# nmwsharp/diffusion-net

Hardware: AMD Instinct MI355X
Metric: vertices/sec fwd+bwd, C_width=128 K=128 (higher is better)
Workload: dtype f32; 1 GPU; train step (fwd+NLL+bwd+Adam) on a ragged batch of 16 meshes x ~10000 vertices per GPU, DiffusionNet C_in=3 C_out=8 C_width=128 K=128 N_block=4 outputs_at=faces dropout=on; meshes_per_gpu=16, verts_per_gpu_step=158481, parallelism=dp1, streams_per_gpu=1, step_mode=HIP-graph replay

## Files before the change

diffusion-net_amd/csrc/dn_tn_da.hip:

```cpp
#include "dn_common.h"
#include <string.h>

#define DN_DA_THREADS 512
#define DN_DA_KS 16
#define DN_DA_ROWB 576
#define DN_DA_PLANE (DN_DA_KS * DN_DA_ROWB)
#define DN_DA_BUF (6 * DN_DA_PLANE)
#define DN_DA_LDS (128 * 1024)

struct DaRegs {
    float4 dd, gx, gy;
    float live;
};

__device__ __forceinline__ void da_load(const DaArgs& g, long long r_beg, long long r_end, int step, int kr, int q, DaRegs& R) {
    const long long row = r_beg + (long long)step * DN_DA_KS + kr;
    const bool ok = row < r_end;
    const long long off = (ok ? row : r_beg) * 128 + 4 * q;
    R.live = ok ? 1.f : 0.f;
    R.dd = *reinterpret_cast<const float4*>(g.dd + off);
    R.gx = *reinterpret_cast<const float4*>(g.gx + off);
    R.gy = *reinterpret_cast<const float4*>(g.gy + off);
}

template <int NP>
__device__ __forceinline__ void da_put(unsigned char* planes, int off, float4 v, float s) {
    uint2 pl[NP];
    dn_split_f4<NP>(v, s, pl);
#pragma unroll
    for (int p = 0; p < NP; ++p) *reinterpret_cast<uint2*>(planes + p * DN_DA_PLANE + off) = pl[p];
}

template <int NP>
__device__ __forceinline__ void da_store(unsigned char* buf, int kr, int q, const DaRegs& R, float sa, float sb) {
    const float4 bx = dn_f4_scale(R.gx, R.live), by = dn_f4_scale(R.gy, R.live);
    const float4 ax = dn_f4_mul(R.dd, bx), ay = dn_f4_mul(R.dd, by);
    const int off = kr * DN_DA_ROWB + q * 8;
    da_put<NP>(buf, off, ax, sa);
    da_put<NP>(buf, off + 256, ay, sa);
    da_put<NP>(buf + 3 * DN_DA_PLANE, off, bx, sb);
    da_put<NP>(buf + 3 * DN_DA_PLANE, off + 256, by, sb);
}

__device__ __forceinline__ uint4 da_frag(const unsigned char* p) {
    const uint2 lo = dn_lds_tr16(p), hi = dn_lds_tr16(p + 4 * DN_DA_ROWB);
    return make_uint4(lo.x, lo.y, hi.x, hi.y);
}

template <int NP>
__device__ __forceinline__ void da_compute(const unsigned char* buf, int wr, int wc, int lane, f32x16 (&acc)[4][2]) {
    const int g = lane >> 4, c = lane & 15;
    const int lane_off = (8 * (g >> 1) + (c >> 2)) * DN_DA_ROWB + (16 * (g & 1) + 4 * (c & 3)) * 2;
    const unsigned char* sA = buf + lane_off + wr * 256;
    const unsigned char* sB = buf + 3 * DN_DA_PLANE + lane_off + wc * 128;
    uint4 b[NP][2];
#pragma unroll
    for (int p = 0; p < NP; ++p)
#pragma unroll
        for (int nt = 0; nt < 2; ++nt) b[p][nt] = da_frag(sB + p * DN_DA_PLANE + nt * 64);
#pragma unroll
    for (int mt = 0; mt < 4; ++mt) {
        uint4 a[NP];
#pragma unroll
        for (int p = 0; p < NP; ++p) a[p] = da_frag(sA + p * DN_DA_PLANE + mt * 64);
        constexpr int NPROD = NP == 3 ? 6 : 3;
        constexpr int PA[6] = {NP == 3 ? 1 : 0, NP == 3 ? 0 : 1, NP == 3 ? 2 : 0, 0, 1, 0};
        constexpr int PB[6] = {1, NP == 3 ? 2 : 0, 0, 1, 0, 0};
#pragma unroll
        for (int p = 0; p < NPROD; ++p)
#pragma unroll
            for (int nt = 0; nt < 2; ++nt) {
                if constexpr (NP == 3) acc[mt][nt] = dn_mfma_bf16(a[PA[p]], b[PB[p]][nt], acc[mt][nt]);
                else acc[mt][nt] = dn_mfma_f16(a[PA[p]], b[PB[p]][nt], acc[mt][nt]);
            }
    }
}

DN_CLK_DECLARE(tn_da)
template <int NP>
__global__ __launch_bounds__(DN_DA_THREADS) DN_WAVES_PER_EU(2) void tngemm_da_kernel(DaArgs g) {
    DN_CLK_STAMP(tn_da, 0);
    float sa = 1.f, sb = 1.f, so = 1.f;
    if constexpr (NP == 2) {
        sa = dn_pow2_scale(dn_amax_eval(g.a_amax));
        sb = dn_pow2_scale(dn_amax_eval(g.b_amax));
        so = (1.f / sa) * (1.f / sb);
    }
    DN_DYN_SMEM(smem_raw);
    unsigned char* smem = reinterpret_cast<unsigned char*>(smem_raw);
    const int tid = threadIdx.x, lane = tid & 63, wave = tid >> 6;
    const int wr = wave >> 2, wc = wave & 3;
    const int kr = tid >> 5, q = tid & 31;

    const long long r_beg = (long long)blockIdx.x * g.rows_per_wg;
    const long long r_end = (r_beg + g.rows_per_wg < g.V) ? r_beg + g.rows_per_wg : g.V;
    const int nsteps = r_end > r_beg ? (int)((r_end - r_beg + DN_DA_KS - 1) / DN_DA_KS) : 0;

    f32x16 acc[4][2];
#pragma unroll
    for (int i = 0; i < 4; ++i)
#pragma unroll
        for (int j = 0; j < 2; ++j)
#pragma unroll
            for (int r = 0; r < 16; ++r) acc[i][j][r] = 0.f;

    if (nsteps > 0) {
        DaRegs R0, R1;
        da_load(g, r_beg, r_end, 0, kr, q, R0);
        da_load(g, r_beg, r_end, 1, kr, q, R1);
        da_store<NP>(smem, kr, q, R0, sa, sb);
        da_load(g, r_beg, r_end, 2, kr, q, R0);
        __syncthreads();
        for (int s = 0; s < nsteps; s += 2) {
            da_store<NP>(smem + DN_DA_BUF, kr, q, R1, sa, sb);
            da_load(g, r_beg, r_end, s + 3, kr, q, R1);
            da_compute<NP>(smem, wr, wc, lane, acc);
            __syncthreads();
            if (s + 1 < nsteps) {
                da_store<NP>(smem, kr, q, R0, sa, sb);
                da_load(g, r_beg, r_end, s + 4, kr, q, R0);
                da_compute<NP>(smem + DN_DA_BUF, wr, wc, lane, acc);
                __syncthreads();
            }
        }
    }
    __syncthreads();

    float* ex = reinterpret_cast<float*>(smem);
    if (wc >= 2) {
        float* mine = ex + (size_t)(wr * 2 + (wc - 2)) * 8 * 16 * 64;
#pragma unroll
        for (int mt = 0; mt < 4; ++mt)
#pragma unroll
            for (int nt = 0; nt < 2; ++nt)
#pragma unroll
                for (int r = 0; r < 16; ++r) mine[((mt * 2 + nt) * 16 + r) * 64 + lane] = acc[mt][nt][r];
    }
    __syncthreads();
    if (wc < 2) {
        const float* theirs = ex + (size_t)((1 - wr) * 2 + wc) * 8 * 16 * 64;
        const float sgn = wr == 0 ? 1.f : -1.f;
        float* out = g.partial + ((long long)blockIdx.x * 2 + wr) * 128 * 128;
        const int li = lane & 31;
#pragma unroll
        for (int mt = 0; mt < 4; ++mt)
#pragma unroll
            for (int nt = 0; nt < 2; ++nt)
#pragma unroll
                for (int r = 0; r < 16; ++r) {
                    const int o = mt * 32 + dn_acc_row(r, lane), c = wc * 64 + nt * 32 + li;
                    const float v = acc[mt][nt][r] + sgn * theirs[((mt * 2 + nt) * 16 + r) * 64 + lane];
                    out[o * 128 + c] = NP == 2 ? v * so : v;
                }
    }
    DN_CLK_STAMP(tn_da, 1);
}

int dn_launch_tn_da(const float* dd, const float* gx, const float* gy, long long V, float* partial, int nwg, hipStream_t stream,
                    const float* dd_amax, const float* g_amax) {
    if (V <= 0 || nwg <= 0) return DN_ERR_BAD_MODE;
    DaArgs g;
    memset(&g, 0, sizeof(g));
    g.dd = dd; g.gx = gx; g.gy = gy; g.partial = partial; g.V = V;
    g.f16 = (dd_amax && g_amax) ? 1 : 0;
    g.a_amax.p[0] = dd_amax; g.a_amax.mul = g_amax; g.b_amax.p[0] = g_amax;
    const long long per = (V + nwg - 1) / nwg;
    g.rows_per_wg = (int)((per + DN_DA_KS - 1) / DN_DA_KS * DN_DA_KS);
#ifndef DN_EMULATE
    static unsigned long long lds_opt_in = 0;
    { const int oe_ = dn_lds_opt_in(reinterpret_cast<const void*>(&tngemm_da_kernel<3>), DN_DA_LDS, &lds_opt_in); if (oe_) return oe_; }
    static unsigned long long lds_opt_in2 = 0;
    { const int oe_ = dn_lds_opt_in(reinterpret_cast<const void*>(&tngemm_da_kernel<2>), DN_DA_LDS, &lds_opt_in2); if (oe_) return oe_; }
#endif
    dn_prof_begin(DN_K_TN_DA, stream);
    if (g.f16) DN_LAUNCH(tngemm_da_kernel<2>, dim3(nwg, 1, 1), dim3(DN_DA_THREADS, 1, 1), DN_DA_LDS, stream, g);
    else DN_LAUNCH(tngemm_da_kernel<3>, dim3(nwg, 1, 1), dim3(DN_DA_THREADS, 1, 1), DN_DA_LDS, stream, g);
    dn_prof_end(DN_K_TN_DA, stream, 8.0 * (double)V * 128.0 * 128.0, 4.0 * (3.0 * (double)V * 128.0 + 2.0 * nwg * 128.0 * 128.0));
    return (int)hipGetLastError();
}
```

diffusion-net_amd/csrc/dn_tn_tiles.h:

```cpp
#pragma once
#include "dn_common.h"

enum { DN_TN_PLAIN = 0, DN_TN_ROWSCALE = 1, DN_TN_COLSUM = 2, DN_TN_QA = 3 };

#define DN_TX_THREADS 512
#define DN_TX_ROWB 320
#define DN_TX_PLANE (DN_KB * DN_TX_ROWB)

struct TxRegs {
    float4 a[2], b[2], qa[2];
    float ma[2], mb[2];
};

template <int FLAVOR>
__device__ __forceinline__ void tx_load(const TnArgs& g, const DnTile& ch, int step, int kr0, bool a_ok, bool b_ok,
                                        const float* ap, const float* aq, int ald, const float* bp, int bld, TxRegs& R) {
#pragma unroll
    for (int i = 0; i < 2; ++i) {
        const int kr = step * DN_KB + kr0 + 16 * i;
        const bool kok = kr < ch.nrows;
        const long long row = (long long)ch.row0 + (kok ? kr : 0);
        R.ma[i] = (kok && a_ok) ? 1.f : 0.f;
        R.mb[i] = (kok && b_ok) ? 1.f : 0.f;
        R.a[i] = *reinterpret_cast<const float4*>(ap + row * ald);
        R.b[i] = *reinterpret_cast<const float4*>(bp + row * bld);
        if (FLAVOR == DN_TN_QA) R.qa[i] = *reinterpret_cast<const float4*>(aq + row * ald);
        if (FLAVOR == DN_TN_ROWSCALE) R.qa[i].x = g.b_rowscale[row];
    }
}

template <int NP = 3>
__device__ __forceinline__ void tx_put(unsigned char* planes, int off, float4 v, float s = 1.f) {
    uint2 pl[NP];
    dn_split_f4<NP>(v, s, pl);
#pragma unroll
    for (int p = 0; p < NP; ++p) *reinterpret_cast<uint2*>(planes + p * DN_TX_PLANE + off) = pl[p];
}

template <int FLAVOR, int NP = 3>
__device__ __forceinline__ void tx_store(unsigned char* sA, unsigned char* sB, int kr0, int q, const TxRegs& R, float4& csum,
                                         float sa = 1.f, float sb = 1.f) {
#pragma unroll
    for (int i = 0; i < 2; ++i) {
        float4 va = dn_f4_scale(R.a[i], R.ma[i]);
        const float4 vb = dn_f4_scale(R.b[i], FLAVOR == DN_TN_ROWSCALE ? R.mb[i] * R.qa[i].x : R.mb[i]);
        if (FLAVOR == DN_TN_QA) va = dn_f4_mul(va, R.qa[i]);
        if (FLAVOR == DN_TN_COLSUM) { csum.x += va.x; csum.y += va.y; csum.z += va.z; csum.w += va.w; }
        const int off = (kr0 + 16 * i) * DN_TX_ROWB + q * 8;
        tx_put<NP>(sA, off, va, sa);
        tx_put<NP>(sB, off, vb, sb);
    }
}

__device__ __forceinline__ uint4 tx_frag(const unsigned char* p) {
    const uint2 lo = dn_lds_tr16(p), hi = dn_lds_tr16(p + 4 * DN_TX_ROWB);
    return make_uint4(lo.x, lo.y, hi.x, hi.y);
}

template <int NP = 3>
__device__ __forceinline__ void tx_compute(const unsigned char* sA, const unsigned char* sB, int wr, int wc, int lane,
                                           f32x16 (&acc)[2]) {
    const int g = lane >> 4, c = lane & 15;
    const int lane_off = (8 * (g >> 1) + (c >> 2)) * DN_TX_ROWB + (16 * (g & 1) + 4 * (c & 3)) * 2;
#pragma unroll
    for (int s = 0; s < 2; ++s) {
        uint4 a[NP][2], b[NP];
#pragma unroll
        for (int p = 0; p < NP; ++p) {
            const int base = p * DN_TX_PLANE + s * 16 * DN_TX_ROWB + lane_off;
#pragma unroll
            for (int mt = 0; mt < 2; ++mt) a[p][mt] = tx_frag(sA + base + (wr * 64 + mt * 32) * 2);
            b[p] = tx_frag(sB + base + (wc * 32) * 2);
        }
        constexpr int NPROD = NP == 3 ? 6 : 3;
        constexpr int PA[6] = {NP == 3 ? 1 : 0, NP == 3 ? 0 : 1, NP == 3 ? 2 : 0, 0, 1, 0};
        constexpr int PB[6] = {1, NP == 3 ? 2 : 0, 0, 1, 0, 0};
#pragma unroll
        for (int p = 0; p < NPROD; ++p)
#pragma unroll
            for (int mt = 0; mt < 2; ++mt) {
                if constexpr (NP == 3) acc[mt] = dn_mfma_bf16(a[PA[p]][mt], b[PB[p]], acc[mt]);
                else acc[mt] = dn_mfma_f16(a[PA[p]][mt], b[PB[p]], acc[mt]);
            }
    }
}
```

diffusion-net_amd/csrc/dn_tngemm.hip:

```cpp
#include "dn_tn_tiles.h"
#include <string.h>

#define DN_TO 128

__device__ __forceinline__ float tn_elem(const TnSeg* s, int ns, long long row, int col) {
    int c = col;
    for (int i = 0; i < ns; ++i) {
        if (c < s[i].w) {
            const long long off = row * s[i].ld + c;
            float v = s[i].p[off];
            if (s[i].q) v *= s[i].q[off];
            return v;
        }
        c -= s[i].w;
    }
    return 0.f;
}


struct TnRegs {
    float4 a[4], b[4], qa[4];
    float ma[4], mb[4];
};

template <bool ALIGNED, int FLAVOR>
__device__ __forceinline__ void tn_load(const TnArgs& g, const DnTile& ch, int step, int kr0, int acol, int bcol, bool a_ok,
                                        bool b_ok, const float* ap, const float* aq, int ald, const float* bp, int bld,
                                        TnRegs& R) {
    if (ALIGNED) {
#pragma unroll
        for (int i = 0; i < 4; ++i) {
            const int kr = step * DN_KB + kr0 + 8 * i;
            const bool kok = kr < ch.nrows;
            const long long row = (long long)ch.row0 + (kok ? kr : 0);
            R.ma[i] = (kok && a_ok) ? 1.f : 0.f;
            R.mb[i] = (kok && b_ok) ? 1.f : 0.f;
            R.a[i] = *reinterpret_cast<const float4*>(ap + row * ald);
            R.b[i] = *reinterpret_cast<const float4*>(bp + row * bld);
            if (FLAVOR == DN_TN_QA) R.qa[i] = *reinterpret_cast<const float4*>(aq + row * ald);
            if (FLAVOR == DN_TN_ROWSCALE) R.qa[i].x = g.b_rowscale[row];
        }
    } else {
#pragma unroll
        for (int i = 0; i < 4; ++i) {
            const int kr = step * DN_KB + kr0 + 8 * i;
            const long long row = (long long)ch.row0 + kr;
            float e[4] = {0.f, 0.f, 0.f, 0.f}, f[4] = {0.f, 0.f, 0.f, 0.f};
            if (kr < ch.nrows) {
                const float rs = g.b_rowscale ? g.b_rowscale[row] : 1.f;
#pragma unroll
                for (int c = 0; c < 4; ++c) {
                    if (acol + c < g.M) e[c] = tn_elem(g.a, g.na, row, acol + c);
                    if (bcol + c < g.N) f[c] = tn_elem(g.b, g.nb, row, bcol + c) * rs;
                }
            }
            R.a[i] = make_float4(e[0], e[1], e[2], e[3]);
            R.b[i] = make_float4(f[0], f[1], f[2], f[3]);
            R.ma[i] = 1.f;
            R.mb[i] = 1.f;
            if (FLAVOR == DN_TN_QA) R.qa[i] = make_float4(1.f, 1.f, 1.f, 1.f);
            if (FLAVOR == DN_TN_ROWSCALE) R.qa[i].x = 1.f;
        }
    }
}

template <int FLAVOR>
__device__ __forceinline__ void tn_store(float* sA, float* sB, int kr0, int q, const TnRegs& R, float4& csum) {
#pragma unroll
    for (int i = 0; i < 4; ++i) {
        float4 va = dn_f4_scale(R.a[i], R.ma[i]);
        float4 vb = dn_f4_scale(R.b[i], FLAVOR == DN_TN_ROWSCALE ? R.mb[i] * R.qa[i].x : R.mb[i]);
        if (FLAVOR == DN_TN_QA) va = dn_f4_mul(va, R.qa[i]);
        if (FLAVOR == DN_TN_COLSUM) { csum.x += va.x; csum.y += va.y; csum.z += va.z; csum.w += va.w; }
        const int kr = kr0 + 8 * i;
        *reinterpret_cast<float4*>(&sA[kr * DN_TO + 4 * q]) = va;
        *reinterpret_cast<float4*>(&sB[kr * DN_TO + 4 * q]) = vb;
    }
}

__device__ __forceinline__ void tn_compute(const float* sA, const float* sB, int wr, int wc, int li, int ls, f32x16 (&acc)[2][2]) {
#pragma unroll
    for (int kg = 0; kg < 4; ++kg) {
        float af[2][4], bf[2][4];
#pragma unroll
        for (int t = 0; t < 4; ++t) {
            const int kr = 8 * kg + 4 * ls + t;
#pragma unroll
            for (int i = 0; i < 2; ++i) {
                af[i][t] = sA[kr * DN_TO + (wr * 2 + i) * 32 + li];
                bf[i][t] = sB[kr * DN_TO + (wc * 2 + i) * 32 + li];
            }
        }
#pragma unroll
        for (int t = 0; t < 4; ++t)
#pragma unroll
            for (int i = 0; i < 2; ++i)
#pragma unroll
                for (int j = 0; j < 2; ++j) acc[i][j] = dn_mfma(af[i][t], bf[j][t], acc[i][j]);
    }
}

template <bool ALIGNED, int FLAVOR>
__global__ __launch_bounds__(256) void tngemm_kernel(TnArgs g) {
    constexpr int SBUF = 2 * DN_KB * DN_TO;
    DN_DYN_SMEM(smem_raw);
    float* smem = reinterpret_cast<float*>(smem_raw);

    const int tid = threadIdx.x, lane = tid & 63, wave = tid >> 6;
    const int wr = wave >> 1, wc = wave & 1;
    const int li = lane & 31, ls = lane >> 5;
    const int n0 = blockIdx.y * DN_TO, m0 = blockIdx.z * DN_TO;
    const bool do_colsum = FLAVOR == DN_TN_COLSUM && blockIdx.y == 0;
    const bool wave_active = (m0 + wr * 64 < g.M) && (n0 + wc * 64 < g.N);

    f32x16 acc[2][2];
#pragma unroll
    for (int i = 0; i < 2; ++i)
#pragma unroll
        for (int j = 0; j < 2; ++j)
#pragma unroll
            for (int r = 0; r < 16; ++r) acc[i][j][r] = 0.f;

    const int q = tid & 31, kr0 = tid >> 5;
    const int acol = m0 + 4 * q, bcol = n0 + 4 * q;
    const float* ap = g.a[0].p; const float* aq = g.a[0].q ? g.a[0].q : g.a[0].p; int ald = g.a[0].ld;
    const float* bp = g.b[0].p; int bld = g.b[0].ld;
    const bool a_ok = acol < g.M, b_ok = bcol < g.N;
    if (ALIGNED) {
        int c = acol;
        for (int i = 0; i < g.na; ++i) {
            if (a_ok && c >= 0 && c < g.a[i].w) { ap = g.a[i].p + c; aq = (g.a[i].q ? g.a[i].q : g.a[i].p) + c; ald = g.a[i].ld; }
            c -= g.a[i].w;
        }
        c = bcol;
        for (int i = 0; i < g.nb; ++i) {
            if (b_ok && c >= 0 && c < g.b[i].w) { bp = g.b[i].p + c; bld = g.b[i].ld; }
            c -= g.b[i].w;
        }
    }
    float4 csum = dn_f4_zero();
    TnRegs R;

    const int c_beg = blockIdx.x * g.group;
    const int c_end = (c_beg + g.group < g.nchunks) ? c_beg + g.group : g.nchunks;
    for (int ci = c_beg; ci < c_end; ++ci) {
        const DnTile ch = g.chunks[ci];
        const int nsteps = (ch.nrows + DN_KB - 1) / DN_KB;
        tn_load<ALIGNED, FLAVOR>(g, ch, 0, kr0, acol, bcol, a_ok, b_ok, ap, aq, ald, bp, bld, R);
        tn_store<FLAVOR>(smem, smem + DN_KB * DN_TO, kr0, q, R, csum);
        if (nsteps > 1) tn_load<ALIGNED, FLAVOR>(g, ch, 1, kr0, acol, bcol, a_ok, b_ok, ap, aq, ald, bp, bld, R);
        __syncthreads();
        int st = 0;
        for (; st + 2 < nsteps; ++st) {
            float* cur = smem + (st & 1) * SBUF;
            float* nxt = smem + ((st & 1) ^ 1) * SBUF;
            tn_store<FLAVOR>(nxt, nxt + DN_KB * DN_TO, kr0, q, R, csum);
            tn_load<ALIGNED, FLAVOR>(g, ch, st + 2, kr0, acol, bcol, a_ok, b_ok, ap, aq, ald, bp, bld, R);
            tn_compute(cur, cur + DN_KB * DN_TO, wr, wc, li, ls, acc);
            __syncthreads();
        }
        if (st + 1 < nsteps) {
            float* cur = smem + (st & 1) * SBUF;
            float* nxt = smem + ((st & 1) ^ 1) * SBUF;
            tn_store<FLAVOR>(nxt, nxt + DN_KB * DN_TO, kr0, q, R, csum);
            tn_compute(cur, cur + DN_KB * DN_TO, wr, wc, li, ls, acc);
            __syncthreads();
            ++st;
        }
        {
            float* cur = smem + (st & 1) * SBUF;
            tn_compute(cur, cur + DN_KB * DN_TO, wr, wc, li, ls, acc);
            __syncthreads();
        }
    }
    float* out = g.partial + (long long)blockIdx.x * g.M * g.N;
#pragma unroll
    for (int i = 0; i < 2; ++i)
#pragma unroll
        for (int j = 0; j < 2; ++j) {
            if (!wave_active) continue;
            const int n = n0 + (wc * 2 + j) * 32 + li;
#pragma unroll
            for (int r = 0; r < 16; ++r) {
                const int m = m0 + (wr * 2 + i) * 32 + dn_acc_row(r, lane);
                if (m < g.M && n < g.N) out[(long long)m * g.N + n] = acc[i][j][r];
            }
        }
    if (do_colsum) {
        *reinterpret_cast<float4*>(&smem[kr0 * DN_TO + 4 * q]) = csum;
        __syncthreads();
        if (tid < DN_TO && m0 + tid < g.M) {
            float sum = 0.f;
#pragma unroll
            for (int k = 0; k < 8; ++k) sum += smem[k * DN_TO + tid];
            g.colsum[(long long)blockIdx.x * g.M + m0 + tid] = sum;
        }
    }
}

template <bool ALIGNED, int FLAVOR>
static int tn_launch(const TnArgs& g, dim3 grid, hipStream_t stream) {
    const size_t smem = (size_t)2 * 2 * DN_KB * DN_TO * sizeof(float);
    DN_LAUNCH((tngemm_kernel<ALIGNED, FLAVOR>), grid, dim3(256, 1, 1), smem, stream, g);
    return (int)hipGetLastError();
}

template <int FLAVOR, int NP>
__device__ __forceinline__ void tn_x3_body(const TnArgs& g, const int bx, const int by, const int bz) {
    float sa = 1.f, sb = 1.f, so = 1.f;
    if constexpr (NP == 2) {
        sa = dn_pow2_scale(dn_amax_eval(g.a_amax));
        sb = dn_pow2_scale(dn_amax_eval(g.b_amax));
        so = (1.f / sa) * (1.f / sb);
    }

    constexpr int SBUF = 6 * DN_TX_PLANE;
    DN_DYN_SMEM(smem_raw);
    unsigned char* smem = reinterpret_cast<unsigned char*>(smem_raw);

    const int tid = threadIdx.x, lane = tid & 63, wave = tid >> 6;
    const int wr = wave >> 2, wc = wave & 3;
    const int li = lane & 31;
    const int n0 = by * DN_TO, m0 = bz * DN_TO;
    const bool do_colsum = FLAVOR == DN_TN_COLSUM && by == 0;
    const bool wave_active = (m0 + wr * 64 < g.M) && (n0 + wc * 32 < g.N);

    f32x16 acc[2];
#pragma unroll
    for (int i = 0; i < 2; ++i)
#pragma unroll
        for (int r = 0; r < 16; ++r) acc[i][r] = 0.f;

    const int q = tid & 31, kr0 = tid >> 5;
    const int acol = m0 + 4 * q, bcol = n0 + 4 * q;
    const float* ap = g.a[0].p; const float* aq = g.a[0].q ? g.a[0].q : g.a[0].p; int ald = g.a[0].ld;
    const float* bp = g.b[0].p; int bld = g.b[0].ld;
    const bool a_ok = acol < g.M, b_ok = bcol < g.N;
    {
        int c = acol;
        for (int i = 0; i < g.na; ++i) {
            if (a_ok && c >= 0 && c < g.a[i].w) { ap = g.a[i].p + c; aq = (g.a[i].q ? g.a[i].q : g.a[i].p) + c; ald = g.a[i].ld; }
            c -= g.a[i].w;
        }
        c = bcol;
        for (int i = 0; i < g.nb; ++i) {
            if (b_ok && c >= 0 && c < g.b[i].w) { bp = g.b[i].p + c; bld = g.b[i].ld; }
            c -= g.b[i].w;
        }
    }
    float4 csum = dn_f4_zero();
    TxRegs R;

    const int c_beg = bx * g.group;
    const int c_end = (c_beg + g.group < g.nchunks) ? c_beg + g.group : g.nchunks;
    for (int ci = c_beg; ci < c_end; ++ci) {
        const DnTile ch = g.chunks[ci];
        const int nsteps = (ch.nrows + DN_KB - 1) / DN_KB;
        tx_load<FLAVOR>(g, ch, 0, kr0, a_ok, b_ok, ap, aq, ald, bp, bld, R);
        tx_store<FLAVOR, NP>(smem, smem + 3 * DN_TX_PLANE, kr0, q, R, csum, sa, sb);
        __syncthreads();
        for (int st = 0; st < nsteps; ++st) {
            if (st + 1 < nsteps) tx_load<FLAVOR>(g, ch, st + 1, kr0, a_ok, b_ok, ap, aq, ald, bp, bld, R);
            tx_compute<NP>(smem, smem + 3 * DN_TX_PLANE, wr, wc, lane, acc);
            __syncthreads();
            if (st + 1 < nsteps) {
                tx_store<FLAVOR, NP>(smem, smem + 3 * DN_TX_PLANE, kr0, q, R, csum, sa, sb);
                __syncthreads();
            }
        }
    }
    float* out = g.partial + (long long)bx * g.M * g.N;
    if (wave_active) {
        const int n = n0 + wc * 32 + li;
#pragma unroll
        for (int i = 0; i < 2; ++i)
#pragma unroll
            for (int r = 0; r < 16; ++r) {
                const int m = m0 + (wr * 2 + i) * 32 + dn_acc_row(r, lane);
                if (m < g.M && n < g.N) out[(long long)m * g.N + n] = NP == 2 ? acc[i][r] * so : acc[i][r];
            }
    }
    if (do_colsum) {
        float* red = reinterpret_cast<float*>(smem);
        *reinterpret_cast<float4*>(&red[kr0 * DN_TO + 4 * q]) = csum;
        __syncthreads();
        if (tid < DN_TO && m0 + tid < g.M) {
            float sum = 0.f;
#pragma unroll
            for (int k = 0; k < 16; ++k) sum += red[k * DN_TO + tid];
            g.colsum[(long long)bx * g.M + m0 + tid] = sum;
        }
    }
}

template <int FLAVOR, int NP>
__global__ __launch_bounds__(DN_TX_THREADS, 4) void tngemm_x3_kernel(TnArgs g) {
    int bx = blockIdx.x, by = blockIdx.y, bz = blockIdx.z;
    if (g.lin_ny > 0) {
        const int nt = g.lin_ny * g.lin_nz, nb = g.lin_nb, local = (int)blockIdx.x, nfull = nb & ~7;
        int tile;
        if (local < nfull * nt) { const int seq = local >> 3; bx = 8 * (seq / nt) + (local & 7); tile = seq % nt; }
        else { const int t = local - nfull * nt, rem = nb - nfull; bx = nfull + t % rem; tile = t / rem; }
        by = tile % g.lin_ny; bz = tile / g.lin_ny;
    }
    tn_x3_body<FLAVOR, NP>(g, bx, by, bz);
}
#define DN_TN_MULTI 3
struct TnMulti { TnArgs p[DN_TN_MULTI]; int first[DN_TN_MULTI + 1]; int nblk[DN_TN_MULTI]; int ny[DN_TN_MULTI]; int count; };
DN_CLK_DECLARE(tn_multi)
template <int FLAVOR, int NP>
__global__ __launch_bounds__(DN_TX_THREADS, 4) void tngemm_x3_multi_kernel(TnMulti mm) {
    DN_CLK_STAMP(tn_multi, 0);
    int pi = 0;
#pragma unroll
    for (int i = 1; i < DN_TN_MULTI; ++i) pi = (i < mm.count && (int)blockIdx.x >= mm.first[i]) ? i : pi;
    const int local = (int)blockIdx.x - mm.first[pi];
    if (pi == 0) tn_x3_body<FLAVOR, NP>(mm.p[0], local % mm.nblk[0], (local / mm.nblk[0]) % mm.ny[0], local / (mm.nblk[0] * mm.ny[0]));
    else if (pi == 1) tn_x3_body<FLAVOR, NP>(mm.p[1], local % mm.nblk[1], (local / mm.nblk[1]) % mm.ny[1], local / (mm.nblk[1] * mm.ny[1]));
    else tn_x3_body<FLAVOR, NP>(mm.p[2], local % mm.nblk[2], (local / mm.nblk[2]) % mm.ny[2], local / (mm.nblk[2] * mm.ny[2]));
    DN_CLK_STAMP(tn_multi, 1);
}

template <int FLAVOR, int NP>
static int tx_launch_np(const TnArgs& g, dim3 grid, hipStream_t stream) {
    const size_t smem = (size_t)6 * DN_TX_PLANE;
#ifndef DN_EMULATE
    static unsigned long long lds_opt_in = 0;
    { const int oe_ = dn_lds_opt_in(reinterpret_cast<const void*>(&tngemm_x3_kernel<FLAVOR, NP>), smem, &lds_opt_in); if (oe_) return oe_; }
#endif
    DN_LAUNCH((tngemm_x3_kernel<FLAVOR, NP>), grid, dim3(DN_TX_THREADS, 1, 1), smem, stream, g);
    return (int)hipGetLastError();
}
template <int FLAVOR>
static int tx_launch(const TnArgs& g, dim3 grid, hipStream_t stream) {
    return g.f16 ? tx_launch_np<FLAVOR, 2>(g, grid, stream) : tx_launch_np<FLAVOR, 3>(g, grid, stream);
}


int dn_launch_tngemm(const TnArgs& g_in, int nchunks, hipStream_t stream) {
    if (nchunks <= 0 || g_in.M <= 0 || g_in.N <= 0) return 0;
    TnArgs g = g_in;
    g.nchunks = nchunks;
    if (g.group < 1) g.group = 1;
    const int nblk = (nchunks + g.group - 1) / g.group;
    dim3 grid(nblk, (g.N + DN_TO - 1) / DN_TO, (g.M + DN_TO - 1) / DN_TO);
    bool has_qa = false;
    for (int i = 0; i < g.na; ++i) has_qa = has_qa || g.a[i].q != nullptr;
    for (int i = 0; i < g.nb; ++i) if (g.b[i].q) return DN_ERR_BAD_MODE;
    const int flavor = has_qa ? DN_TN_QA : (g.colsum ? DN_TN_COLSUM : (g.b_rowscale ? DN_TN_ROWSCALE : DN_TN_PLAIN));
    if ((has_qa && (g.colsum || g.b_rowscale)) || (g.colsum && g.b_rowscale)) return DN_ERR_BAD_MODE;
    const double rows = g.acct_rows;
    dn_prof_begin(DN_K_TNGEMM, stream);
    int err;
    if (g.aligned) {
        g.lin_nb = g.lin_ny = g.lin_nz = 0;
        if (grid.y * grid.z > 1) {
            g.lin_nb = nblk; g.lin_ny = (int)grid.y; g.lin_nz = (int)grid.z;
            grid = dim3(nblk * grid.y * grid.z, 1, 1);
        }
        switch (flavor) {
            case DN_TN_QA: err = tx_launch<DN_TN_QA>(g, grid, stream); break;
            case DN_TN_COLSUM: err = tx_launch<DN_TN_COLSUM>(g, grid, stream); break;
            case DN_TN_ROWSCALE: err = tx_launch<DN_TN_ROWSCALE>(g, grid, stream); break;
            default: err = tx_launch<DN_TN_PLAIN>(g, grid, stream); break;
        }
    } else {
        switch (flavor) {
            case DN_TN_QA: err = tn_launch<false, DN_TN_QA>(g, grid, stream); break;
            case DN_TN_COLSUM: err = tn_launch<false, DN_TN_COLSUM>(g, grid, stream); break;
            case DN_TN_ROWSCALE: err = tn_launch<false, DN_TN_ROWSCALE>(g, grid, stream); break;
            default: err = tn_launch<false, DN_TN_PLAIN>(g, grid, stream); break;
        }
    }
    dn_prof_end(DN_K_TNGEMM, stream, 2.0 * rows * g.M * g.N,
                4.0 * (rows * (g.M + g.N) + (double)nblk * g.M * g.N));
    return err;
}

int dn_launch_tngemm_multi(const TnArgs* gs, const int* nchunks, int count, hipStream_t stream) {
    if (count <= 0) return 0;
    bool ok = count <= DN_TN_MULTI;
    for (int i = 0; i < count && ok; ++i) {
        const TnArgs& g = gs[i];
        bool has_qa = false;
        for (int k = 0; k < g.na; ++k) has_qa = has_qa || g.a[k].q != nullptr;
        ok = g.aligned && !g.f16 && !has_qa && g.colsum && !g.b_rowscale && nchunks[i] > 0 && g.M > 0 && g.N > 0;
    }
    if (!ok || count == 1) {
        for (int i = 0; i < count; ++i) { const int e = dn_launch_tngemm(gs[i], nchunks[i], stream); if (e) return e; }
        return 0;
    }
    TnMulti mm;
    memset(&mm, 0, sizeof(mm));
    mm.count = count;
    double flops = 0.0, bytes = 0.0;
    int total = 0;
    for (int i = 0; i < count; ++i) {
        mm.p[i] = gs[i];
        mm.p[i].nchunks = nchunks[i];
        if (mm.p[i].group < 1) mm.p[i].group = 1;
        mm.nblk[i] = (nchunks[i] + mm.p[i].group - 1) / mm.p[i].group;
        mm.ny[i] = (gs[i].N + DN_TO - 1) / DN_TO;
        const int nz = (gs[i].M + DN_TO - 1) / DN_TO;
        mm.first[i] = total;
        total += mm.nblk[i] * mm.ny[i] * nz;
        const double rows = gs[i].acct_rows;
        flops += 2.0 * rows * gs[i].M * gs[i].N;
        bytes += 4.0 * (rows * (gs[i].M + gs[i].N) + (double)mm.nblk[i] * gs[i].M * gs[i].N);
    }
    mm.first[count] = total;
    const size_t smem = (size_t)6 * DN_TX_PLANE;
#ifndef DN_EMULATE
    static unsigned long long lds_opt_in = 0;
    { const int oe_ = dn_lds_opt_in(reinterpret_cast<const void*>(&tngemm_x3_multi_kernel<DN_TN_COLSUM, 3>), smem, &lds_opt_in); if (oe_) return oe_; }
#endif
    dn_prof_begin(DN_K_TN_MULTI, stream);
    DN_LAUNCH((tngemm_x3_multi_kernel<DN_TN_COLSUM, 3>), dim3(total, 1, 1), dim3(DN_TX_THREADS, 1, 1), smem, stream, mm);
    dn_prof_end(DN_K_TN_MULTI, stream, flops, bytes);
    return (int)hipGetLastError();
}
```

Measured before the change: 32.73 million vertices/s.

## Interleave LDS staging and global loads with MFMA in TN GEMM kernels

The da kernel now splits the next-tile LDS store into quarters and issues one per m-tile between MFMA groups, with the global prefetch placed in the last slot. A-fragments are double-buffered across m-tiles. The multi-launch x3 TN GEMM gets a ping-pong path: it stages each half k-slice into the same LDS tile while MFMAs run on the other half. Scheduling barriers keep the compiler from regrouping the stores and loads. The aim is to hide LDS write and global-load latency behind matrix math. The cost is more registers, more barriers, and a subtle LDS reuse pattern that could race or lower occupancy.

```diff
diff --git a/diffusion-net_amd/csrc/dn_tn_da.hip b/diffusion-net_amd/csrc/dn_tn_da.hip
--- a/diffusion-net_amd/csrc/dn_tn_da.hip
+++ b/diffusion-net_amd/csrc/dn_tn_da.hip
@@ -1,4 +1,4 @@
-#include "dn_common.h"
+#include "dn_tn_tiles.h"
 #include <string.h>
 
 #define DN_DA_THREADS 512
@@ -32,14 +32,17 @@
 }
 
 template <int NP>
+__device__ __forceinline__ void da_store_quarter(unsigned char* buf, int kr, int q, int qtr, const DaRegs& R, float sa, float sb) {
+    const float4 b = dn_f4_scale((qtr & 1) ? R.gy : R.gx, R.live);
+    const int off = kr * DN_DA_ROWB + q * 8 + (qtr & 1) * 256;
+    if (qtr < 2) da_put<NP>(buf, off, dn_f4_mul(R.dd, b), sa);
+    else da_put<NP>(buf + 3 * DN_DA_PLANE, off, b, sb);
+}
+
+template <int NP>
 __device__ __forceinline__ void da_store(unsigned char* buf, int kr, int q, const DaRegs& R, float sa, float sb) {
-    const float4 bx = dn_f4_scale(R.gx, R.live), by = dn_f4_scale(R.gy, R.live);
-    const float4 ax = dn_f4_mul(R.dd, bx), ay = dn_f4_mul(R.dd, by);
-    const int off = kr * DN_DA_ROWB + q * 8;
-    da_put<NP>(buf, off, ax, sa);
-    da_put<NP>(buf, off + 256, ay, sa);
-    da_put<NP>(buf + 3 * DN_DA_PLANE, off, bx, sb);
-    da_put<NP>(buf + 3 * DN_DA_PLANE, off + 256, by, sb);
+#pragma unroll
+    for (int qtr = 0; qtr < 4; ++qtr) da_store_quarter<NP>(buf, kr, q, qtr, R, sa, sb);
 }
 
 __device__ __forceinline__ uint4 da_frag(const unsigned char* p) {
@@ -48,21 +51,29 @@
 }
 
 template <int NP>
-__device__ __forceinline__ void da_compute(const unsigned char* buf, int wr, int wc, int lane, f32x16 (&acc)[4][2]) {
-    const int g = lane >> 4, c = lane & 15;
-    const int lane_off = (8 * (g >> 1) + (c >> 2)) * DN_DA_ROWB + (16 * (g & 1) + 4 * (c & 3)) * 2;
-    const unsigned char* sA = buf + lane_off + wr * 256;
-    const unsigned char* sB = buf + 3 * DN_DA_PLANE + lane_off + wc * 128;
-    uint4 b[NP][2];
+__device__ __forceinline__ void da_step(const unsigned char* cur, unsigned char* nxt, const DaArgs& g, long long r_beg, long long r_end,
+                                        int ld_step, int kr, int q, DaRegs& R, float sa, float sb, int wr, int wc, int lane,
+                                        f32x16 (&acc)[4][2]) {
+    const int lg = lane >> 4, c = lane & 15;
+    const int lane_off = (8 * (lg >> 1) + (c >> 2)) * DN_DA_ROWB + (16 * (lg & 1) + 4 * (c & 3)) * 2;
+    const unsigned char* sA = cur + lane_off + wr * 256;
+    const unsigned char* sB = cur + 3 * DN_DA_PLANE + lane_off + wc * 128;
+    uint4 b[NP][2], a[2][NP];
 #pragma unroll
     for (int p = 0; p < NP; ++p)
 #pragma unroll
         for (int nt = 0; nt < 2; ++nt) b[p][nt] = da_frag(sB + p * DN_DA_PLANE + nt * 64);
 #pragma unroll
+    for (int p = 0; p < NP; ++p) a[0][p] = da_frag(sA + p * DN_DA_PLANE);
+#pragma unroll
     for (int mt = 0; mt < 4; ++mt) {
-        uint4 a[NP];
+        if (mt > 0) DN_SCHED_FENCE();
+        da_store_quarter<NP>(nxt, kr, q, mt, R, sa, sb);
+        if (mt == 3) da_load(g, r_beg, r_end, ld_step, kr, q, R);
+        if (mt < 3) {
 #pragma unroll
-        for (int p = 0; p < NP; ++p) a[p] = da_frag(sA + p * DN_DA_PLANE + mt * 64);
+            for (int p = 0; p < NP; ++p) a[(mt + 1) & 1][p] = da_frag(sA + p * DN_DA_PLANE + (mt + 1) * 64);
+        }
         constexpr int NPROD = NP == 3 ? 6 : 3;
         constexpr int PA[6] = {NP == 3 ? 1 : 0, NP == 3 ? 0 : 1, NP == 3 ? 2 : 0, 0, 1, 0};
         constexpr int PB[6] = {1, NP == 3 ? 2 : 0, 0, 1, 0, 0};
@@ -70,8 +81,8 @@
         for (int p = 0; p < NPROD; ++p)
 #pragma unroll
             for (int nt = 0; nt < 2; ++nt) {
-                if constexpr (NP == 3) acc[mt][nt] = dn_mfma_bf16(a[PA[p]], b[PB[p]][nt], acc[mt][nt]);
-                else acc[mt][nt] = dn_mfma_f16(a[PA[p]], b[PB[p]][nt], acc[mt][nt]);
+                if constexpr (NP == 3) acc[mt][nt] = dn_mfma_bf16(a[mt & 1][PA[p]], b[PB[p]][nt], acc[mt][nt]);
+                else acc[mt][nt] = dn_mfma_f16(a[mt & 1][PA[p]], b[PB[p]][nt], acc[mt][nt]);
             }
     }
 }
@@ -112,14 +123,10 @@
         da_load(g, r_beg, r_end, 2, kr, q, R0);
         __syncthreads();
         for (int s = 0; s < nsteps; s += 2) {
-            da_store<NP>(smem + DN_DA_BUF, kr, q, R1, sa, sb);
-            da_load(g, r_beg, r_end, s + 3, kr, q, R1);
-            da_compute<NP>(smem, wr, wc, lane, acc);
+            da_step<NP>(smem, smem + DN_DA_BUF, g, r_beg, r_end, s + 3, kr, q, R1, sa, sb, wr, wc, lane, acc);
             __syncthreads();
             if (s + 1 < nsteps) {
-                da_store<NP>(smem, kr, q, R0, sa, sb);
-                da_load(g, r_beg, r_end, s + 4, kr, q, R0);
-                da_compute<NP>(smem + DN_DA_BUF, wr, wc, lane, acc);
+                da_step<NP>(smem + DN_DA_BUF, smem, g, r_beg, r_end, s + 4, kr, q, R0, sa, sb, wr, wc, lane, acc);
                 __syncthreads();
             }
         }
diff --git a/diffusion-net_amd/csrc/dn_tn_tiles.h b/diffusion-net_amd/csrc/dn_tn_tiles.h
--- a/diffusion-net_amd/csrc/dn_tn_tiles.h
+++ b/diffusion-net_amd/csrc/dn_tn_tiles.h
@@ -13,20 +13,24 @@
 };
 
 template <int FLAVOR>
+__device__ __forceinline__ void tx_load_half(const TnArgs& g, const DnTile& ch, int step, int i, int kr0, bool a_ok, bool b_ok,
+                                             const float* ap, const float* aq, int ald, const float* bp, int bld, TxRegs& R) {
+    const int kr = step * DN_KB + kr0 + 16 * i;
+    const bool kok = kr < ch.nrows;
+    const long long row = (long long)ch.row0 + (kok ? kr : 0);
+    R.ma[i] = (kok && a_ok) ? 1.f : 0.f;
+    R.mb[i] = (kok && b_ok) ? 1.f : 0.f;
+    R.a[i] = *reinterpret_cast<const float4*>(ap + row * ald);
+    R.b[i] = *reinterpret_cast<const float4*>(bp + row * bld);
+    if (FLAVOR == DN_TN_QA) R.qa[i] = *reinterpret_cast<const float4*>(aq + row * ald);
+    if (FLAVOR == DN_TN_ROWSCALE) R.qa[i].x = g.b_rowscale[row];
+}
+
+template <int FLAVOR>
 __device__ __forceinline__ void tx_load(const TnArgs& g, const DnTile& ch, int step, int kr0, bool a_ok, bool b_ok,
                                         const float* ap, const float* aq, int ald, const float* bp, int bld, TxRegs& R) {
 #pragma unroll
-    for (int i = 0; i < 2; ++i) {
-        const int kr = step * DN_KB + kr0 + 16 * i;
-        const bool kok = kr < ch.nrows;
-        const long long row = (long long)ch.row0 + (kok ? kr : 0);
-        R.ma[i] = (kok && a_ok) ? 1.f : 0.f;
-        R.mb[i] = (kok && b_ok) ? 1.f : 0.f;
-        R.a[i] = *reinterpret_cast<const float4*>(ap + row * ald);
-        R.b[i] = *reinterpret_cast<const float4*>(bp + row * bld);
-        if (FLAVOR == DN_TN_QA) R.qa[i] = *reinterpret_cast<const float4*>(aq + row * ald);
-        if (FLAVOR == DN_TN_ROWSCALE) R.qa[i].x = g.b_rowscale[row];
-    }
+    for (int i = 0; i < 2; ++i) tx_load_half<FLAVOR>(g, ch, step, i, kr0, a_ok, b_ok, ap, aq, ald, bp, bld, R);
 }
 
 template <int NP = 3>
@@ -38,18 +42,29 @@
 }
 
 template <int FLAVOR, int NP = 3>
+__device__ __forceinline__ void tx_store_half_a(unsigned char* sA, int kr0, int q, int i, const TxRegs& R, float4& csum, float sa = 1.f) {
+    float4 va = dn_f4_scale(R.a[i], R.ma[i]);
+    if (FLAVOR == DN_TN_QA) va = dn_f4_mul(va, R.qa[i]);
+    if (FLAVOR == DN_TN_COLSUM) { csum.x += va.x; csum.y += va.y; csum.z += va.z; csum.w += va.w; }
+    tx_put<NP>(sA, (kr0 + 16 * i) * DN_TX_ROWB + q * 8, va, sa);
+}
+template <int FLAVOR, int NP = 3>
+__device__ __forceinline__ void tx_store_half_b(unsigned char* sB, int kr0, int q, int i, const TxRegs& R, float sb = 1.f) {
+    const float4 vb = dn_f4_scale(R.b[i], FLAVOR == DN_TN_ROWSCALE ? R.mb[i] * R.qa[i].x : R.mb[i]);
+    tx_put<NP>(sB, (kr0 + 16 * i) * DN_TX_ROWB + q * 8, vb, sb);
+}
+template <int FLAVOR, int NP = 3>
+__device__ __forceinline__ void tx_store_half(unsigned char* sA, unsigned char* sB, int kr0, int q, int i, const TxRegs& R,
+                                              float4& csum, float sa = 1.f, float sb = 1.f) {
+    tx_store_half_a<FLAVOR, NP>(sA, kr0, q, i, R, csum, sa);
+    tx_store_half_b<FLAVOR, NP>(sB, kr0, q, i, R, sb);
+}
+
+template <int FLAVOR, int NP = 3>
 __device__ __forceinline__ void tx_store(unsigned char* sA, unsigned char* sB, int kr0, int q, const TxRegs& R, float4& csum,
                                          float sa = 1.f, float sb = 1.f) {
 #pragma unroll
-    for (int i = 0; i < 2; ++i) {
-        float4 va = dn_f4_scale(R.a[i], R.ma[i]);
-        const float4 vb = dn_f4_scale(R.b[i], FLAVOR == DN_TN_ROWSCALE ? R.mb[i] * R.qa[i].x : R.mb[i]);
-        if (FLAVOR == DN_TN_QA) va = dn_f4_mul(va, R.qa[i]);
-        if (FLAVOR == DN_TN_COLSUM) { csum.x += va.x; csum.y += va.y; csum.z += va.z; csum.w += va.w; }
-        const int off = (kr0 + 16 * i) * DN_TX_ROWB + q * 8;
-        tx_put<NP>(sA, off, va, sa);
-        tx_put<NP>(sB, off, vb, sb);
-    }
+    for (int i = 0; i < 2; ++i) tx_store_half<FLAVOR, NP>(sA, sB, kr0, q, i, R, csum, sa, sb);
 }
 
 __device__ __forceinline__ uint4 tx_frag(const unsigned char* p) {
@@ -57,30 +72,79 @@
     return make_uint4(lo.x, lo.y, hi.x, hi.y);
 }
 
+__device__ __forceinline__ int tx_lane_off(int lane) {
+    const int g = lane >> 4, c = lane & 15;
+    return (8 * (g >> 1) + (c >> 2)) * DN_TX_ROWB + (16 * (g & 1) + 4 * (c & 3)) * 2;
+}
+
+template <int NP = 3>
+__device__ __forceinline__ void tx_frags_half(const unsigned char* sA, const unsigned char* sB, int wr, int wc, int lane, int h,
+                                              uint4 (&a)[NP][2], uint4 (&b)[NP]) {
+    const int lane_off = tx_lane_off(lane);
+#pragma unroll
+    for (int p = 0; p < NP; ++p) {
+        const int base = p * DN_TX_PLANE + h * 16 * DN_TX_ROWB + lane_off;
+#pragma unroll
+        for (int mt = 0; mt < 2; ++mt) a[p][mt] = tx_frag(sA + base + (wr * 64 + mt * 32) * 2);
+        b[p] = tx_frag(sB + base + (wc * 32) * 2);
+    }
+}
+
+template <int NP = 3, int P0 = 0, int P1 = (NP == 3 ? 6 : 3)>
+__device__ __forceinline__ void tx_mfma_half(const uint4 (&a)[NP][2], const uint4 (&b)[NP], f32x16 (&acc)[2]) {
+    constexpr int PA[6] = {NP == 3 ? 1 : 0, NP == 3 ? 0 : 1, NP == 3 ? 2 : 0, 0, 1, 0};
+    constexpr int PB[6] = {1, NP == 3 ? 2 : 0, 0, 1, 0, 0};
+#pragma unroll
+    for (int p = P0; p < P1; ++p)
+#pragma unroll
+        for (int mt = 0; mt < 2; ++mt) {
+            if constexpr (NP == 3) acc[mt] = dn_mfma_bf16(a[PA[p]][mt], b[PB[p]], acc[mt]);
+            else acc[mt] = dn_mfma_f16(a[PA[p]][mt], b[PB[p]], acc[mt]);
+        }
+}
+
+template <int NP = 3>
+__device__ __forceinline__ void tx_compute_half(const unsigned char* sA, const unsigned char* sB, int wr, int wc, int lane, int h,
+                                                f32x16 (&acc)[2]) {
+    uint4 a[NP][2], b[NP];
+    tx_frags_half<NP>(sA, sB, wr, wc, lane, h, a, b);
+    tx_mfma_half<NP>(a, b, acc);
+}
+
 template <int NP = 3>
 __device__ __forceinline__ void tx_compute(const unsigned char* sA, const unsigned char* sB, int wr, int wc, int lane,
                                            f32x16 (&acc)[2]) {
-    const int g = lane >> 4, c = lane & 15;
-    const int lane_off = (8 * (g >> 1) + (c >> 2)) * DN_TX_ROWB + (16 * (g & 1) + 4 * (c & 3)) * 2;
 #pragma unroll
-    for (int s = 0; s < 2; ++s) {
-        uint4 a[NP][2], b[NP];
-#pragma unroll
-        for (int p = 0; p < NP; ++p) {
-            const int base = p * DN_TX_PLANE + s * 16 * DN_TX_ROWB + lane_off;
-#pragma unroll
-            for (int mt = 0; mt < 2; ++mt) a[p][mt] = tx_frag(sA + base + (wr * 64 + mt * 32) * 2);
-            b[p] = tx_frag(sB + base + (wc * 32) * 2);
-        }
-        constexpr int NPROD = NP == 3 ? 6 : 3;
-        constexpr int PA[6] = {NP == 3 ? 1 : 0, NP == 3 ? 0 : 1, NP == 3 ? 2 : 0, 0, 1, 0};
-        constexpr int PB[6] = {1, NP == 3 ? 2 : 0, 0, 1, 0, 0};
-#pragma unroll
-        for (int p = 0; p < NPROD; ++p)
-#pragma unroll
-            for (int mt = 0; mt < 2; ++mt) {
-                if constexpr (NP == 3) acc[mt] = dn_mfma_bf16(a[PA[p]][mt], b[PB[p]], acc[mt]);
-                else acc[mt] = dn_mfma_f16(a[PA[p]][mt], b[PB[p]], acc[mt]);
-            }
-    }
+    for (int h = 0; h < 2; ++h) tx_compute_half<NP>(sA, sB, wr, wc, lane, h, acc);
 }
+
+#ifdef DN_EMULATE
+#define DN_SCHED_FENCE() do {} while (0)
+#else
+#define DN_SCHED_FENCE() __builtin_amdgcn_sched_barrier(0)
+#endif
+
+template <int FLAVOR, int NP, int HM, bool STAGE>
+__device__ __forceinline__ void tx_phase(unsigned char* sA, unsigned char* sB, const TnArgs& g, const DnTile& ch, int ld_step, int kr0,
+                                         int q, bool a_ok, bool b_ok, const float* ap, const float* aq, int ald, const float* bp,
+                                         int bld, TxRegs& R, float4& csum, float sa, float sb, int wr, int wc, int lane,
+                                         f32x16 (&acc)[2]) {
+    constexpr int NPROD = NP == 3 ? 6 : 3;
+    uint4 a[NP][2], b[NP];
+    tx_frags_half<NP>(sA, sB, wr, wc, lane, HM, a, b);
+    if (!STAGE) { tx_mfma_half<NP>(a, b, acc); return; }
+    constexpr int i = 1 - HM;
+    const bool kok = (ld_step - 1) * DN_KB + kr0 + 16 * i < ch.nrows;
+    R.ma[i] = (kok && a_ok) ? 1.f : 0.f;
+    R.mb[i] = (kok && b_ok) ? 1.f : 0.f;
+    tx_mfma_half<NP, 0, NPROD - 3>(a, b, acc);
+    DN_SCHED_FENCE();
+    tx_store_half_a<FLAVOR, NP>(sA, kr0, q, i, R, csum, sa);
+    tx_mfma_half<NP, NPROD - 3, NPROD - 2>(a, b, acc);
+    DN_SCHED_FENCE();
+    tx_store_half_b<FLAVOR, NP>(sB, kr0, q, i, R, sb);
+    tx_mfma_half<NP, NPROD - 2, NPROD - 1>(a, b, acc);
+    DN_SCHED_FENCE();
+    tx_load_half<FLAVOR>(g, ch, ld_step, i, kr0, a_ok, b_ok, ap, aq, ald, bp, bld, R);
+    tx_mfma_half<NP, NPROD - 1, NPROD>(a, b, acc);
+}
diff --git a/diffusion-net_amd/csrc/dn_tngemm.hip b/diffusion-net_amd/csrc/dn_tngemm.hip
--- a/diffusion-net_amd/csrc/dn_tngemm.hip
+++ b/diffusion-net_amd/csrc/dn_tngemm.hip
@@ -205,7 +205,7 @@
     return (int)hipGetLastError();
 }
 
-template <int FLAVOR, int NP>
+template <int FLAVOR, int NP, bool PINGPONG>
 __device__ __forceinline__ void tn_x3_body(const TnArgs& g, const int bx, const int by, const int bz) {
     float sa = 1.f, sb = 1.f, so = 1.f;
     if constexpr (NP == 2) {
@@ -256,16 +256,37 @@
     for (int ci = c_beg; ci < c_end; ++ci) {
         const DnTile ch = g.chunks[ci];
         const int nsteps = (ch.nrows + DN_KB - 1) / DN_KB;
-        tx_load<FLAVOR>(g, ch, 0, kr0, a_ok, b_ok, ap, aq, ald, bp, bld, R);
-        tx_store<FLAVOR, NP>(smem, smem + 3 * DN_TX_PLANE, kr0, q, R, csum, sa, sb);
-        __syncthreads();
-        for (int st = 0; st < nsteps; ++st) {
-            if (st + 1 < nsteps) tx_load<FLAVOR>(g, ch, st + 1, kr0, a_ok, b_ok, ap, aq, ald, bp, bld, R);
-            tx_compute<NP>(smem, smem + 3 * DN_TX_PLANE, wr, wc, lane, acc);
-            __syncthreads();
-            if (st + 1 < nsteps) {
-                tx_store<FLAVOR, NP>(smem, smem + 3 * DN_TX_PLANE, kr0, q, R, csum, sa, sb);
+        if constexpr (PINGPONG) {
+            unsigned char* sA = smem;
+            unsigned char* sB = smem + 3 * DN_TX_PLANE;
+#define DN_TX_PHASE(HM, STAGE, step) \
+            tx_phase<FLAVOR, NP, HM, STAGE>(sA, sB, g, ch, (step), kr0, q, a_ok, b_ok, ap, aq, ald, bp, bld, R, csum, sa, sb, wr, wc, lane, acc)
+            tx_load<FLAVOR>(g, ch, 0, kr0, a_ok, b_ok, ap, aq, ald, bp, bld, R);
+            tx_store_half<FLAVOR, NP>(sA, sB, kr0, q, 0, R, csum, sa, sb);
+            tx_load_half<FLAVOR>(g, ch, 1, 0, kr0, a_ok, b_ok, ap, aq, ald, bp, bld, R);
+            __syncthreads();
+            DN_TX_PHASE(0, true, 1);
+            __syncthreads();
+            for (int st = 1; st < nsteps; ++st) {
+                DN_TX_PHASE(1, true, st + 1);
                 __syncthreads();
+                DN_TX_PHASE(0, true, st + 1);
+                __syncthreads();
+            }
+            DN_TX_PHASE(1, false, 0);
+#undef DN_TX_PHASE
+        } else {
+            tx_load<FLAVOR>(g, ch, 0, kr0, a_ok, b_ok, ap, aq, ald, bp, bld, R);
+            tx_store<FLAVOR, NP>(smem, smem + 3 * DN_TX_PLANE, kr0, q, R, csum, sa, sb);
+            __syncthreads();
+            for (int st = 0; st < nsteps; ++st) {
+                if (st + 1 < nsteps) tx_load<FLAVOR>(g, ch, st + 1, kr0, a_ok, b_ok, ap, aq, ald, bp, bld, R);
+                tx_compute<NP>(smem, smem + 3 * DN_TX_PLANE, wr, wc, lane, acc);
+                __syncthreads();
+                if (st + 1 < nsteps) {
+                    tx_store<FLAVOR, NP>(smem, smem + 3 * DN_TX_PLANE, kr0, q, R, csum, sa, sb);
+                    __syncthreads();
+                }
             }
         }
     }
@@ -282,6 +303,7 @@
     }
     if (do_colsum) {
         float* red = reinterpret_cast<float*>(smem);
+        if constexpr (PINGPONG) __syncthreads();
         *reinterpret_cast<float4*>(&red[kr0 * DN_TO + 4 * q]) = csum;
         __syncthreads();
         if (tid < DN_TO && m0 + tid < g.M) {
@@ -303,7 +325,7 @@
         else { const int t = local - nfull * nt, rem = nb - nfull; bx = nfull + t % rem; tile = t / rem; }
         by = tile % g.lin_ny; bz = tile / g.lin_ny;
     }
-    tn_x3_body<FLAVOR, NP>(g, bx, by, bz);
+    tn_x3_body<FLAVOR, NP, false>(g, bx, by, bz);
 }
 #define DN_TN_MULTI 3
 struct TnMulti { TnArgs p[DN_TN_MULTI]; int first[DN_TN_MULTI + 1]; int nblk[DN_TN_MULTI]; int ny[DN_TN_MULTI]; int count; };
@@ -315,9 +337,9 @@
 #pragma unroll
     for (int i = 1; i < DN_TN_MULTI; ++i) pi = (i < mm.count && (int)blockIdx.x >= mm.first[i]) ? i : pi;
     const int local = (int)blockIdx.x - mm.first[pi];
-    if (pi == 0) tn_x3_body<FLAVOR, NP>(mm.p[0], local % mm.nblk[0], (local / mm.nblk[0]) % mm.ny[0], local / (mm.nblk[0] * mm.ny[0]));
-    else if (pi == 1) tn_x3_body<FLAVOR, NP>(mm.p[1], local % mm.nblk[1], (local / mm.nblk[1]) % mm.ny[1], local / (mm.nblk[1] * mm.ny[1]));
-    else tn_x3_body<FLAVOR, NP>(mm.p[2], local % mm.nblk[2], (local / mm.nblk[2]) % mm.ny[2], local / (mm.nblk[2] * mm.ny[2]));
+    if (pi == 0) tn_x3_body<FLAVOR, NP, true>(mm.p[0], local % mm.nblk[0], (local / mm.nblk[0]) % mm.ny[0], local / (mm.nblk[0] * mm.ny[0]));
+    else if (pi == 1) tn_x3_body<FLAVOR, NP, true>(mm.p[1], local % mm.nblk[1], (local / mm.nblk[1]) % mm.ny[1], local / (mm.nblk[1] * mm.ny[1]));
+    else tn_x3_body<FLAVOR, NP, true>(mm.p[2], local % mm.nblk[2], (local / mm.nblk[2]) % mm.ny[2], local / (mm.nblk[2] * mm.ny[2]));
     DN_CLK_STAMP(tn_multi, 1);
 }
 
```

New measurement: 32.79 million vertices/s, median of 6. About the same (+0.2%).
